# wolearyc/ramannoodle

Hardware: AMD Instinct MI355X
Metric: structures/sec (GNN polarizability eval) (higher is better)
Workload: dtype f32

## Files before the change

ramannoodle_amd/csrc/kernels_c2_pairs.hip:

```cpp
#include "fused_common.hpp"

namespace rn {

struct C2PairArgs {
  const float *node;
  float *out;
  int64_t M;
  int N, NP;
  const int *pair_a, *pair_b;
  Dims d;
  PassW<float> w;
};

namespace {
constexpr int C2P_THREADS = 256;
}

__global__ __launch_bounds__(C2P_THREADS, 2) void c2_pairs_kernel(C2PairArgs a) {
  __shared__ __attribute__((aligned(16))) float s_bias[2 * FP], s_g1[2 * FP], s_b1[2 * FP], s_g2[FP], s_b2[FP];
  const int tid = threadIdx.x, lane = tid & 63, wave = tid >> 6;
  const int l15 = lane & 15, quad = lane >> 4;
  const float sc2 = a.w.mfma_scale_c[4];
  for (int c = tid; c < 2 * FP; c += C2P_THREADS) {
    s_bias[c] = a.w.c2_bias_c[c] * sc2;
    s_g1[c] = a.w.c2_norm_1.g[c];
    s_b1[c] = a.w.c2_norm_1.b[c];
    if (c < FP) {
      s_g2[c] = a.w.c2_norm_2.g[c];
      s_b2[c] = a.w.c2_norm_2.b[c];
    }
  }
  WaveB<true> bW[4];
#pragma unroll
  for (int p = 0; p < 4; ++p) bW[p].load(a.w.c2_WT_c, 2 * FP, 32 * p, l15, quad, sc2);
  __syncthreads();

  const float inv2n = 1.0f / (float)(2 * a.d.Fe), invn = 1.0f / (float)a.d.Fe;
  const float eps_c2 = 1e-5f * sc2 * sc2;
  const int64_t ntiles = (a.M + 15) / 16, stride = (int64_t)gridDim.x * (C2P_THREADS / 64);

  f32x4 xb[4], xa[4];
  auto fetch = [&](int64_t tile) {
    int64_t row = tile * 16 + l15;
    if (row >= a.M) row = a.M - 1;
    const int64_t s = row / a.NP;
    const int p = (int)(row - s * a.NP);
    const float *nb = a.node + (s * a.N + a.pair_b[p]) * FP + 16 * quad, *na = a.node + (s * a.N + a.pair_a[p]) * FP + 16 * quad;
#pragma unroll
    for (int j = 0; j < 4; ++j) {
      xb[j] = *reinterpret_cast<const f32x4 *>(nb + 4 * j);
      xa[j] = *reinterpret_cast<const f32x4 *>(na + 4 * j);
    }
  };
  int64_t tile = (int64_t)blockIdx.x * (C2P_THREADS / 64) + wave;
  if (tile < ntiles) fetch(tile);
  for (; tile < ntiles; tile += stride) {
    float af[KS];
#pragma unroll
    for (int j = 0; j < 4; ++j) {
      const f32x4 pr = xb[j] * xa[j];
#pragma unroll
      for (int i = 0; i < 4; ++i) af[4 * j + i] = pr[i];
    }
    f16x8 ah[2], al[2];
    split_f16x8(af, ah[0], al[0]);
    split_f16x8(af + 8, ah[1], al[1]);
    if (tile + stride < ntiles) fetch(tile + stride);

    const int lq = launder(lane >> 4);
    f32x4 acc[4][2];
#pragma unroll
    for (int p = 0; p < 4; ++p) {
#pragma unroll
      for (int t = 0; t < 2; ++t) acc[p][t] = *reinterpret_cast<const f32x4 *>(s_bias + 32 * p + 16 * t + 4 * lq);
      bW[p].product_split(ah, al, acc[p]);
    }
    float q = 0.f;
#pragma unroll
    for (int p = 0; p < 4; ++p)
#pragma unroll
      for (int t = 0; t < 2; ++t)
#pragma unroll
        for (int i = 0; i < 4; ++i) q = fmaf(acc[p][t][i], acc[p][t][i], q);
    q = sum_xor32(sum_xor16(q));
    const float rstd2 = fast_rsq(q * inv2n + eps_c2);
    float gv[2][2][4], sum = 0.f;
#pragma unroll
    for (int p = 0; p < 2; ++p)
#pragma unroll
      for (int t = 0; t < 2; ++t) {
        const int c = 32 * p + 16 * t + 4 * lq;
        const Vec4<float> gf = load4<float>(s_g1 + c), bf = load4<float>(s_b1 + c);
        const Vec4<float> gc = load4<float>(s_g1 + FP + c), bc = load4<float>(s_b1 + FP + c);
#pragma unroll
        for (int i = 0; i < 4; ++i) {
          gv[p][t][i] = gate(acc[p][t][i] * rstd2 * gf.v[i] + bf.v[i], acc[p + 2][t][i] * rstd2 * gc.v[i] + bc.v[i]);
          sum += gv[p][t][i];
        }
      }
    const float mean = sum_xor32(sum_xor16(sum)) * invn;
    float qq = 0.f;
#pragma unroll
    for (int p = 0; p < 2; ++p)
#pragma unroll
      for (int t = 0; t < 2; ++t)
#pragma unroll
        for (int i = 0; i < 4; ++i) {
          const int c = 32 * p + 16 * t + 4 * lq + i;
          gv[p][t][i] = c < a.d.Fe ? gv[p][t][i] - mean : 0.f;
          qq = fmaf(gv[p][t][i], gv[p][t][i], qq);
        }
    const float rstd = fast_rsq(sum_xor32(sum_xor16(qq)) * invn + 1e-5f);
    const int64_t row = tile * 16 + l15 < a.M ? tile * 16 + l15 : a.M - 1;
    {
#pragma unroll
      for (int p = 0; p < 2; ++p)
#pragma unroll
        for (int t = 0; t < 2; ++t) {
          const int c = 32 * p + 16 * t + 4 * lq;
          const Vec4<float> g2 = load4<float>(s_g2 + c), b2 = load4<float>(s_b2 + c);
          f32x4 y;
#pragma unroll
          for (int i = 0; i < 4; ++i) y[i] = gv[p][t][i] * rstd * g2.v[i] + b2.v[i];
          *reinterpret_cast<f32x4 *>(a.out + row * FP + c) = y;
        }
    }
  }
}

void launch_c2_pairs(const float *node, float *out, int S, const Graph &g, Dims d, const PassW<float> &w, hipStream_t st) {
  const int64_t M = (int64_t)S * g.NP;
  if (M == 0) return;
  C2PairArgs a{node, out, M, g.N, g.NP, g.pair_a, g.pair_b, d, w};
  static int cus = 0;
  if (cus == 0) {
    int dev = 0;
    hipDeviceProp_t prop;
    if (hipGetDevice(&dev) == hipSuccess && hipGetDeviceProperties(&prop, dev) == hipSuccess) cus = prop.multiProcessorCount;
    if (cus <= 0) cus = 256;
  }
  const int64_t ntiles = (M + 15) / 16, per_wg = C2P_THREADS / 64;
  const int64_t grid = std::min<int64_t>((ntiles + per_wg - 1) / per_wg, (int64_t)2 * cus);
  c2_pairs_kernel<<<(unsigned)grid, C2P_THREADS, 0, st>>>(a);
}

}
```

Baseline: 67160.

## Pipeline pair index lookup and split, fold gate constants, template padding mask

Replaces per-tile 64-bit division for the (structure, pair) index with incremental advancement, and software-pipelines the pair index lookup, node fetch and f16 split one iteration ahead. It folds the log2e scaling into the norm gamma/beta so the gate runs as exp2/rcp on packed f32x2 math with a clamp. The padding mask becomes a template parameter, so the unpadded case skips the compare. These changes aim to cut integer and transcendental ALU work and hide gather latency, at the cost of more live registers and a more complex pipeline.

Measured after the change: 67480, median of 6. No clear change (+0.5%).

```diff
diff --git a/ramannoodle_amd/csrc/kernels_c2_pairs.hip b/ramannoodle_amd/csrc/kernels_c2_pairs.hip
--- a/ramannoodle_amd/csrc/kernels_c2_pairs.hip
+++ b/ramannoodle_amd/csrc/kernels_c2_pairs.hip
@@ -6,7 +6,7 @@
   const float *node;
   float *out;
   int64_t M;
-  int N, NP;
+  int S, N, NP;
   const int *pair_a, *pair_b;
   Dims d;
   PassW<float> w;
@@ -16,15 +16,17 @@
 constexpr int C2P_THREADS = 256;
 }
 
+template <bool PAD>
 __global__ __launch_bounds__(C2P_THREADS, 2) void c2_pairs_kernel(C2PairArgs a) {
   __shared__ __attribute__((aligned(16))) float s_bias[2 * FP], s_g1[2 * FP], s_b1[2 * FP], s_g2[FP], s_b2[FP];
   const int tid = threadIdx.x, lane = tid & 63, wave = tid >> 6;
   const int l15 = lane & 15, quad = lane >> 4;
   const float sc2 = a.w.mfma_scale_c[4];
   for (int c = tid; c < 2 * FP; c += C2P_THREADS) {
+    const float k = c < FP ? -kLog2e : 2.0f * kLog2e;
     s_bias[c] = a.w.c2_bias_c[c] * sc2;
-    s_g1[c] = a.w.c2_norm_1.g[c];
-    s_b1[c] = a.w.c2_norm_1.b[c];
+    s_g1[c] = k * a.w.c2_norm_1.g[c];
+    s_b1[c] = k * a.w.c2_norm_1.b[c];
     if (c < FP) {
       s_g2[c] = a.w.c2_norm_2.g[c];
       s_b2[c] = a.w.c2_norm_2.b[c];
@@ -37,24 +39,47 @@
 
   const float inv2n = 1.0f / (float)(2 * a.d.Fe), invn = 1.0f / (float)a.d.Fe;
   const float eps_c2 = 1e-5f * sc2 * sc2;
+  const float kClamp = 15.0f * 2.0f * kLog2e;
   const int64_t ntiles = (a.M + 15) / 16, stride = (int64_t)gridDim.x * (C2P_THREADS / 64);
-
+  const int fe_q = a.d.Fe - 4 * quad;
+  int64_t tile = (int64_t)blockIdx.x * (C2P_THREADS / 64) + wave;
+  const int step_rows = (int)stride * 16;
+  const int ds = step_rows / a.NP, dp = step_rows - ds * a.NP;
+  int s, p;
+  {
+    const int64_t row = min(tile * 16 + l15, a.M - 1);
+    s = (int)(row / a.NP);
+    p = (int)(row - (int64_t)s * a.NP);
+  }
+  auto advance = [&]() {
+    p += dp;
+    s += ds;
+    if (p >= a.NP) {
+      p -= a.NP;
+      ++s;
+    }
+    if (s >= a.S) {
+      s = a.S - 1;
+      p = a.NP - 1;
+    }
+  };
+  const float *node_q = a.node + 16 * quad;
   f32x4 xb[4], xa[4];
-  auto fetch = [&](int64_t tile) {
-    int64_t row = tile * 16 + l15;
-    if (row >= a.M) row = a.M - 1;
-    const int64_t s = row / a.NP;
-    const int p = (int)(row - s * a.NP);
-    const float *nb = a.node + (s * a.N + a.pair_b[p]) * FP + 16 * quad, *na = a.node + (s * a.N + a.pair_a[p]) * FP + 16 * quad;
+  int ia, ib;
+  auto lookup = [&]() {
+    ia = a.pair_a[p];
+    ib = a.pair_b[p];
+  };
+  auto fetch = [&]() {
+    const float *nb = node_q + ((int64_t)s * a.N + ib) * FP, *na = node_q + ((int64_t)s * a.N + ia) * FP;
 #pragma unroll
     for (int j = 0; j < 4; ++j) {
       xb[j] = *reinterpret_cast<const f32x4 *>(nb + 4 * j);
       xa[j] = *reinterpret_cast<const f32x4 *>(na + 4 * j);
     }
   };
-  int64_t tile = (int64_t)blockIdx.x * (C2P_THREADS / 64) + wave;
-  if (tile < ntiles) fetch(tile);
-  for (; tile < ntiles; tile += stride) {
+  f16x8 ah[2], al[2];
+  auto split = [&]() {
     float af[KS];
 #pragma unroll
     for (int j = 0; j < 4; ++j) {
@@ -62,76 +87,104 @@
 #pragma unroll
       for (int i = 0; i < 4; ++i) af[4 * j + i] = pr[i];
     }
-    f16x8 ah[2], al[2];
     split_f16x8(af, ah[0], al[0]);
     split_f16x8(af + 8, ah[1], al[1]);
-    if (tile + stride < ntiles) fetch(tile + stride);
+  };
+  lookup();
+  fetch();
+  float *orow = a.out + ((int64_t)s * a.NP + p) * FP;
+  advance();
+  lookup();
+  split();
+  asm volatile("" : "+v"(ia), "+v"(ib));
+  for (; tile < ntiles; tile += stride) {
+    float *const onext = a.out + ((int64_t)s * a.NP + p) * FP;
+    fetch();
+    advance();
+    lookup();
 
     const int lq = launder(lane >> 4);
     f32x4 acc[4][2];
 #pragma unroll
-    for (int p = 0; p < 4; ++p) {
-#pragma unroll
-      for (int t = 0; t < 2; ++t) acc[p][t] = *reinterpret_cast<const f32x4 *>(s_bias + 32 * p + 16 * t + 4 * lq);
-      bW[p].product_split(ah, al, acc[p]);
+    for (int p4 = 0; p4 < 4; ++p4) {
+#pragma unroll
+      for (int t = 0; t < 2; ++t) acc[p4][t] = *reinterpret_cast<const f32x4 *>(s_bias + 32 * p4 + 16 * t + 4 * lq);
+      bW[p4].product_split(ah, al, acc[p4]);
     }
     float q = 0.f;
 #pragma unroll
-    for (int p = 0; p < 4; ++p)
+    for (int p4 = 0; p4 < 4; ++p4)
 #pragma unroll
       for (int t = 0; t < 2; ++t)
 #pragma unroll
-        for (int i = 0; i < 4; ++i) q = fmaf(acc[p][t][i], acc[p][t][i], q);
+        for (int i = 0; i < 4; ++i) q = fmaf(acc[p4][t][i], acc[p4][t][i], q);
     q = sum_xor32(sum_xor16(q));
     const float rstd2 = fast_rsq(q * inv2n + eps_c2);
-    float gv[2][2][4], sum = 0.f;
-#pragma unroll
-    for (int p = 0; p < 2; ++p)
+    const f32x2 rs2 = {rstd2, rstd2}, one2 = {1.0f, 1.0f};
+    f32x4 gv[2][2];
+    float sum = 0.f;
+#pragma unroll
+    for (int p2 = 0; p2 < 2; ++p2)
 #pragma unroll
       for (int t = 0; t < 2; ++t) {
-        const int c = 32 * p + 16 * t + 4 * lq;
-        const Vec4<float> gf = load4<float>(s_g1 + c), bf = load4<float>(s_b1 + c);
-        const Vec4<float> gc = load4<float>(s_g1 + FP + c), bc = load4<float>(s_b1 + FP + c);
-#pragma unroll
-        for (int i = 0; i < 4; ++i) {
-          gv[p][t][i] = gate(acc[p][t][i] * rstd2 * gf.v[i] + bf.v[i], acc[p + 2][t][i] * rstd2 * gc.v[i] + bc.v[i]);
-          sum += gv[p][t][i];
+        const int c = 32 * p2 + 16 * t + 4 * lq;
+        const f32x4 gf = *reinterpret_cast<const f32x4 *>(s_g1 + c), bf = *reinterpret_cast<const f32x4 *>(s_b1 + c);
+        const f32x4 gc = *reinterpret_cast<const f32x4 *>(s_g1 + FP + c), bc = *reinterpret_cast<const f32x4 *>(s_b1 + FP + c);
+#pragma unroll
+        for (int hh = 0; hh < 2; ++hh) {
+          const f32x2 xf = (hh ? acc[p2][t].hi : acc[p2][t].lo) * rs2, xc = (hh ? acc[p2 + 2][t].hi : acc[p2 + 2][t].lo) * rs2;
+          const f32x2 yf = __builtin_elementwise_fma(xf, hh ? gf.hi : gf.lo, hh ? bf.hi : bf.lo);
+          const f32x2 yc = __builtin_elementwise_fma(xc, hh ? gc.hi : gc.lo, hh ? bc.hi : bc.lo);
+          const f32x2 e1 = {fast_exp2(yf.x), fast_exp2(yf.y)};
+          const f32x2 e2 = {fast_exp2(__builtin_amdgcn_fmed3f(yc.x, -kClamp, kClamp)), fast_exp2(__builtin_amdgcn_fmed3f(yc.y, -kClamp, kClamp))};
+          const f32x2 t2 = e2 + one2;
+          const f32x2 den = __builtin_elementwise_fma(e1, t2, t2);
+          const f32x2 rd = {fast_rcp(den.x), fast_rcp(den.y)};
+          const f32x2 g = (e2 - one2) * rd;
+          gv[p2][t][2 * hh] = g.x;
+          gv[p2][t][2 * hh + 1] = g.y;
+          sum += g.x;
+          sum += g.y;
         }
       }
     const float mean = sum_xor32(sum_xor16(sum)) * invn;
     float qq = 0.f;
 #pragma unroll
-    for (int p = 0; p < 2; ++p)
-#pragma unroll
-      for (int t = 0; t < 2; ++t)
+    for (int p2 = 0; p2 < 2; ++p2)
+#pragma unroll
+      for (int t = 0; t < 2; ++t) {
+        gv[p2][t] -= mean;
 #pragma unroll
         for (int i = 0; i < 4; ++i) {
-          const int c = 32 * p + 16 * t + 4 * lq + i;
-          gv[p][t][i] = c < a.d.Fe ? gv[p][t][i] - mean : 0.f;
-          qq = fmaf(gv[p][t][i], gv[p][t][i], qq);
+          if (PAD && 32 * p2 + 16 * t + i >= fe_q) gv[p2][t][i] = 0.f;
+          qq = fmaf(gv[p2][t][i], gv[p2][t][i], qq);
         }
+      }
     const float rstd = fast_rsq(sum_xor32(sum_xor16(qq)) * invn + 1e-5f);
-    const int64_t row = tile * 16 + l15 < a.M ? tile * 16 + l15 : a.M - 1;
-    {
-#pragma unroll
-      for (int p = 0; p < 2; ++p)
-#pragma unroll
-        for (int t = 0; t < 2; ++t) {
-          const int c = 32 * p + 16 * t + 4 * lq;
-          const Vec4<float> g2 = load4<float>(s_g2 + c), b2 = load4<float>(s_b2 + c);
-          f32x4 y;
-#pragma unroll
-          for (int i = 0; i < 4; ++i) y[i] = gv[p][t][i] * rstd * g2.v[i] + b2.v[i];
-          *reinterpret_cast<f32x4 *>(a.out + row * FP + c) = y;
-        }
-    }
+    f32x4 y[2][2];
+#pragma unroll
+    for (int p2 = 0; p2 < 2; ++p2)
+#pragma unroll
+      for (int t = 0; t < 2; ++t) {
+        const int c = 32 * p2 + 16 * t + 4 * lq;
+        const f32x4 g2 = *reinterpret_cast<const f32x4 *>(s_g2 + c), b2 = *reinterpret_cast<const f32x4 *>(s_b2 + c);
+        y[p2][t] = __builtin_elementwise_fma(gv[p2][t] * rstd, g2, b2);
+      }
+    __builtin_amdgcn_sched_barrier(0);
+    split();
+    asm volatile("" : "+v"(ah[0]), "+v"(al[0]), "+v"(ah[1]), "+v"(al[1]), "+v"(ia), "+v"(ib)::"memory");
+#pragma unroll
+    for (int p2 = 0; p2 < 2; ++p2)
+#pragma unroll
+      for (int t = 0; t < 2; ++t) *reinterpret_cast<f32x4 *>(orow + 32 * p2 + 16 * t + 4 * lq) = y[p2][t];
+    orow = onext;
   }
 }
 
 void launch_c2_pairs(const float *node, float *out, int S, const Graph &g, Dims d, const PassW<float> &w, hipStream_t st) {
   const int64_t M = (int64_t)S * g.NP;
   if (M == 0) return;
-  C2PairArgs a{node, out, M, g.N, g.NP, g.pair_a, g.pair_b, d, w};
+  C2PairArgs a{node, out, M, S, g.N, g.NP, g.pair_a, g.pair_b, d, w};
   static int cus = 0;
   if (cus == 0) {
     int dev = 0;
@@ -141,7 +194,8 @@
   }
   const int64_t ntiles = (M + 15) / 16, per_wg = C2P_THREADS / 64;
   const int64_t grid = std::min<int64_t>((ntiles + per_wg - 1) / per_wg, (int64_t)2 * cus);
-  c2_pairs_kernel<<<(unsigned)grid, C2P_THREADS, 0, st>>>(a);
-}
-
-}
+  auto kern = d.Fe != d.FeP ? &c2_pairs_kernel<true> : &c2_pairs_kernel<false>;
+  kern<<<(unsigned)grid, C2P_THREADS, 0, st>>>(a);
+}
+
+}
```
